# carlozamu/dynamic-video-compression-surveillance

Hardware: NVIDIA B200
Metric: 1080p_frames_per_second (higher is better)
Workload: dtype u8

## Files before the change

dynamic_video_compression_surveillance_b200/csrc/k_degrade4p.cuh:

```cuda
#pragma once
#include "k_degrade.cuh"

namespace dvc {

struct QuantP {
    float rcp[3];
    float nqs[3];
    float o[3];
};

template <typename T>
DEVI void dct4_fwd_t(T& x0, T& x1, T& x2, T& x3) {
    const T c1 = splat<T>(DVC_C1), c3 = splat<T>(DVC_C3), nc1 = splat<T>(-DVC_C1);
    const T s0 = add(x0, x3), s1 = add(x1, x2), d0 = sub(x0, x3), d1 = sub(x1, x2);
    x0 = add(s0, s1);
    x2 = sub(s0, s1);
    x1 = fma_(c3, d1, mul(c1, d0));
    x3 = fma_(c3, d0, mul(nc1, d1));
}
template <typename T>
DEVI void dct4_inv_t(T& x0, T& x1, T& x2, T& x3) {
    const T c1 = splat<T>(DVC_C1), c3 = splat<T>(DVC_C3), nc1 = splat<T>(-DVC_C1);
    const T e0 = add(x0, x2), e1 = sub(x0, x2);
    const T o0 = fma_(c3, x3, mul(c1, x1));
// ... 422 lines not shown
        }
    }
    if (counters) {
#pragma unroll
        for (int o = 16; o > 0; o >>= 1) {
            n_motion += __shfl_xor_sync(0xffffffffu, n_motion, o);
            n_static += __shfl_xor_sync(0xffffffffu, n_static, o);
        }
        if ((threadIdx.x & 31) == 0) {
            if (n_motion) atomicAdd(&counters->motion_pixels, (unsigned long long)n_motion);
            if (n_static) atomicAdd(&counters->static_blocks, (unsigned long long)n_static);
        }
    }
}

struct K4Geom {
    int gp;
    int parts;
    int nb;
    int sp;
    int span_bytes;
    int mask_bytes;
};

struct K4SGeom {
    K4Geom g;
    int stages;
    int tiles_per_frame;
    int n_tiles;
    int stage_bytes;
    int ybuf_bytes;
};

constexpr int K4S_GROUPS = 2;
constexpr int K4S_THREADS = K4S_GROUPS * 256 + 32;
constexpr int K4S_ISSUERS = 2;

DEVI void mbar_wait(uint32_t bar, uint32_t parity) {
    uint32_t done = 0;
    while (!done) {
        asm volatile("{\n .reg .pred p;\n mbarrier.try_wait.parity.shared::cta.b64 p, [%1], %2;\n selp.u32 %0, 1, 0, p;\n}"
                     : "=r"(done) : "r"(bar), "r"(parity) : "memory");
    }
}
DEVI void mbar_arrive(uint32_t bar) { asm volatile("mbarrier.arrive.shared::cta.b64 _, [%0];" ::"r"(bar) : "memory"); }
DEVI void group_sync(int id) { asm volatile("bar.sync %0, 256;" ::"r"(id) : "memory"); }

struct K4Walk {
    int f, l, df, dl, tpf;
    DEVI void init(int t0, int step, int tiles_per_frame) {
        tpf = tiles_per_frame; f = t0 / tpf; l = t0 - f * tpf; df = step / tpf; dl = step - df * tpf;
    }
    DEVI void next() { f += df; l += dl; if (l >= tpf) { l -= tpf; ++f; } }
};
struct K4Tile { size_t span_off, mask_off; int nbv, g0, ng; };
DEVI K4Tile k4_tile(const K4Walk& wk, const K4Geom& g, int H, int W, int wpr) {
    const int gpr = W >> 3, nbr = H >> 2;
    K4Tile r;
    int br0;
    if (g.parts == 1) { br0 = wk.l * g.nb; r.nbv = min(g.nb, nbr - br0); r.g0 = 0; r.ng = gpr; }
    else { br0 = wk.l / g.parts; r.nbv = 1; r.g0 = (wk.l - br0 * g.parts) * g.gp; r.ng = min(g.gp, gpr - r.g0); }
    r.span_off = ((size_t)wk.f * H + (size_t)(br0 * 4)) * W * 3 + (size_t)r.g0 * 24;
    r.mask_off = ((size_t)wk.f * H + (size_t)(br0 * 4)) * wpr;
    return r;
}

__global__ void __launch_bounds__(K4S_THREADS, 1)
k_degrade4s(const uint8_t* __restrict__ frames, const uint32_t* __restrict__ over127,
            const uint32_t* __restrict__ nonzero, uint8_t* __restrict__ compressed, uint8_t* __restrict__ overlay,
            int H, int W, int wpr, QuantP qp, Counters* __restrict__ counters, K4SGeom sg) {
    extern __shared__ __align__(128) uint8_t k4_smem[];
    const K4Geom& g = sg.g;
    const uint32_t s0 = (uint32_t)__cvta_generic_to_shared(k4_smem);
    const int S = sg.stages;
    const uint32_t ybufs = s0 + (uint32_t)S * (uint32_t)sg.stage_bytes;
    const uint32_t bars = ybufs + (uint32_t)K4S_GROUPS * (uint32_t)sg.ybuf_bytes;
    const uint32_t desc = (bars + 8u * (uint32_t)(2 * S) + 15u) & ~15u;
    const int tid = threadIdx.x;
    const int first = blockIdx.x, stride = gridDim.x;
    const int nj = first < sg.n_tiles ? (sg.n_tiles - first + stride - 1) / stride : 0;
    const uint32_t pitch = (uint32_t)W * 3u;
    const uint32_t mrow_bytes = (uint32_t)wpr * 4u;
    const bool contiguous = g.parts == 1;

    if (tid == 0) {
        for (int s = 0; s < S; ++s) {
            asm volatile("mbarrier.init.shared::cta.b64 [%0], 1;" ::"r"(bars + 8u * s));
            asm volatile("mbarrier.init.shared::cta.b64 [%0], %1;" ::"r"(bars + 8u * (S + s)), "r"(K4S_ISSUERS));
        }
        asm volatile("fence.mbarrier_init.release.cluster;" ::: "memory");
    }
    __syncthreads();

    if (tid >= K4S_GROUPS * 256) {
        if (tid > K4S_GROUPS * 256) return;
        K4Walk wl;
        wl.init(first, stride, sg.tiles_per_frame);
        for (int j = 0; j < nj; ++j) {
            const int s = j % S;
            const K4Tile t = k4_tile(wl, g, H, W, wpr);
            wl.next();
            const uint32_t sX = s0 + (uint32_t)s * (uint32_t)sg.stage_bytes;
            const uint32_t sMh = sX + g.span_bytes, sMn = sMh + g.mask_bytes;
            const uint32_t full = bars + 8u * s;
            const uint32_t mbytes = (uint32_t)(4 * t.nbv) * mrow_bytes;
            const uint32_t rows = contiguous ? (uint32_t)(4 * t.nbv) : 4u;
            const uint32_t rbytes = contiguous ? pitch : (uint32_t)t.ng * 24u;
            if (j >= S) mbar_wait(bars + 8u * (S + s), (uint32_t)(j / S - 1) & 1u);
            asm volatile("st.shared.v4.b32 [%0], {%1, %2, %3, %4};" ::"r"(desc + 16u * s), "r"(t.nbv), "r"(t.g0), "r"(t.ng), "r"(0) : "memory");
            asm volatile("mbarrier.arrive.expect_tx.shared::cta.b64 _, [%0], %1;" ::"r"(full), "r"(rows * rbytes + 2u * mbytes) : "memory");
            if (contiguous) bulk_load(sX, frames + t.span_off, rows * rbytes, full);
            else
                for (uint32_t r = 0; r < rows; ++r) bulk_load(sX + r * g.sp, frames + t.span_off + (size_t)r * pitch, rbytes, full);
            bulk_load(sMh, over127 + t.mask_off, mbytes, full);
            bulk_load(sMn, nonzero + t.mask_off, mbytes, full);
        }
        return;
    }

    const int grp = tid >> 8, t = tid & 255;
    const bool issuer = t < K4S_ISSUERS;
    const int gpr = W >> 3;
    int brl = 0, gxl = t;
    if (contiguous) { brl = t / gpr; gxl = t - brl * gpr; }
    const uint32_t toff = (uint32_t)(brl * 4) * (uint32_t)g.sp + (uint32_t)gxl * 24u;
    const uint32_t sY = ybufs + (uint32_t)grp * (uint32_t)sg.ybuf_bytes;
    unsigned n_motion = 0, n_static = 0;
    K4Walk ws;
    ws.init(first + grp * stride, K4S_GROUPS * stride, sg.tiles_per_frame);
    int s_prev = -1;
    for (int j = grp; j < nj; j += K4S_GROUPS) {
        const int s = j % S;
        const uint32_t sX = s0 + (uint32_t)s * (uint32_t)sg.stage_bytes;
        const uint32_t sMh = sX + g.span_bytes, sMn = sMh + g.mask_bytes;
        mbar_wait(bars + 8u * s, (uint32_t)(j / S) & 1u);
        uint32_t nbv, tg0, tng, unused;
        asm volatile("ld.shared.v4.b32 {%0, %1, %2, %3}, [%4];" : "=r"(nbv), "=r"(tg0), "=r"(tng), "=r"(unused) : "r"(desc + 16u * s));
        const bool active = brl < (int)nbv && gxl < (int)tng;
        uint32_t w[4][6];
        if (active) {
            const uint32_t moff = (uint32_t)(brl * 4) * mrow_bytes + tg0 + (uint32_t)gxl;
#pragma unroll
            for (int r = 0; r < 4; ++r)
#pragma unroll
                for (int i = 0; i < 3; ++i) lds64(sX + toff + r * g.sp + 8 * i, w[r][2 * i], w[r][2 * i + 1]);
            uint32_t hi[4], nz = 0;
#pragma unroll
            for (int r = 0; r < 4; ++r) {
                hi[r] = lds_u8(sMh + moff + r * mrow_bytes);
                nz |= lds_u8(sMn + moff + r * mrow_bytes);
            }
            if (overlay) {
#pragma unroll
                for (int r = 0; r < 4; ++r) {
                    if (hi[r] == 0u) continue;
                    uint32_t o[6];
#pragma unroll
                    for (int i = 0; i < 6; ++i) o[i] = w[r][i];
#pragma unroll
                    for (int b = 0; b < 2; ++b) {
                        const uint32_t m = hi[r] >> (4 * b);
                        if (m & 1u) { o[3 * b] = (o[3 * b] & 0xff000000u) | 0x00ff0000u; }
                        if (m & 2u) { o[3 * b] &= 0x00ffffffu; o[3 * b + 1] = (o[3 * b + 1] & 0xffff0000u) | 0x0000ff00u; }
                        if (m & 4u) { o[3 * b + 1] &= 0x0000ffffu; o[3 * b + 2] = (o[3 * b + 2] & 0xffffff00u) | 0x000000ffu; }
                        if (m & 8u) { o[3 * b + 2] = (o[3 * b + 2] & 0x000000ffu) | 0xff000000u; }
                    }
#pragma unroll
                    for (int i = 0; i < 3; ++i) sts64(sX + toff + r * g.sp + 8 * i, o[2 * i], o[2 * i + 1]);
                }
            }
            n_motion += __popc(hi[0]) + __popc(hi[1]) + __popc(hi[2]) + __popc(hi[3]);
            const bool st_a = (nz & 0xfu) == 0u, st_b = (nz >> 4) == 0u;
            n_static += (st_a ? 1u : 0u) + (st_b ? 1u : 0u);
            if (compressed) k4_blocks(w, st_a, st_b, qp);
        }
        if (issuer && s_prev >= 0) {
            asm volatile("cp.async.bulk.wait_group.read 0;" ::: "memory");
            mbar_arrive(bars + 8u * (S + s_prev));
        }
        group_sync(1 + grp);
        if (compressed && active) {
#pragma unroll
            for (int r = 0; r < 4; ++r)
#pragma unroll
                for (int i = 0; i < 3; ++i) sts64(sY + toff + r * g.sp + 8 * i, w[r][2 * i], w[r][2 * i + 1]);
        }
        asm volatile("fence.proxy.async.shared::cta;" ::: "memory");
        group_sync(1 + grp);
        if (issuer) {
            uint8_t* dst = t == 0 ? overlay : compressed;
            if (dst) {
                const K4Tile tl = k4_tile(ws, g, H, W, wpr);
                const uint32_t src = t == 0 ? sX : sY;
                if (contiguous) bulk_store(dst + tl.span_off, src, 4u * nbv * pitch);
                else
                    for (uint32_t r = 0; r < 4; ++r) bulk_store(dst + tl.span_off + (size_t)r * pitch, src + r * g.sp, tng * 24u);
            }
            asm volatile("cp.async.bulk.commit_group;" ::: "memory");
            s_prev = s;
        }
        ws.next();
    }
    if (issuer) asm volatile("cp.async.bulk.wait_group.read 0;" ::: "memory");
    if (counters) {
#pragma unroll
        for (int o = 16; o > 0; o >>= 1) {
            n_motion += __shfl_xor_sync(0xffffffffu, n_motion, o);
            n_static += __shfl_xor_sync(0xffffffffu, n_static, o);
        }
        if ((tid & 31) == 0) {
            if (n_motion) atomicAdd(&counters->motion_pixels, (unsigned long long)n_motion);
            if (n_static) atomicAdd(&counters->static_blocks, (unsigned long long)n_static);
        }
    }
}

}
// ... 1 lines not shown
```

dynamic_video_compression_surveillance_b200/csrc/k_mask.cuh:

```cuda
#pragma once
#include "common.cuh"
#include "k_front.cuh"

namespace dvc {

constexpr int WINDOW_MAX = 127;
struct MinCounts { uint8_t v[128]; };

template <int CB>
DEVI void bs_add(uint32_t (&c)[CB], uint32_t x) {
#pragma unroll
    for (int i = 0; i < CB; ++i) { uint32_t t = c[i] & x; c[i] ^= x; x = t; }
}
template <int CB>
DEVI void bs_sub(uint32_t (&c)[CB], uint32_t x) {
#pragma unroll
    for (int i = 0; i < CB; ++i) { uint32_t t = ~c[i] & x; c[i] ^= x; x = t; }
}
template <int CB>
DEVI uint32_t bs_ge(const uint32_t (&c)[CB], uint32_t m) {
    if (m >= (1u << CB)) return 0u;
    uint32_t ge = 0xffffffffu;
#pragma unroll
    for (int i = 0; i < CB; ++i) ge = ((m >> i) & 1u) ? (c[i] & ge) : (c[i] | ge);
    return ge;
}

template <int CNT_BITS>
__global__ void __launch_bounds__(256)
k_window_vote(const uint32_t* __restrict__ ring, int ring_cap, int H, int W, int wpr, long long f0, int slot0, int T,
              int K, const __grid_constant__ MinCounts mc, uint32_t* __restrict__ voted, int seg_len) {
    __shared__ uint8_t s_mc[128];
    if (threadIdx.x < 128) s_mc[threadIdx.x] = mc.v[threadIdx.x];
    __syncthreads();
    const size_t plane_words = (size_t)H * wpr;
    const size_t idx = (size_t)blockIdx.x * blockDim.x + threadIdx.x;
    if (idx >= plane_words) return;
    ring += (size_t)blockIdx.z * ring_cap * plane_words;
    voted += (size_t)blockIdx.z * T * plane_words;
    const int t0 = blockIdx.y * seg_len, t1 = min(T, t0 + seg_len);
    const uint32_t vm = valid_mask((int)(idx % wpr), W);
    uint32_t c[CNT_BITS] = {};
    const long long fs = f0 + t0;
    int s_new = (slot0 + t0) % ring_cap;
    const int nh = (int)min((long long)(K - 1), fs);
    int s = s_new - nh;
    if (s < 0) s += ring_cap;
    for (int i = 0; i < nh; ++i) {
        bs_add(c, ring[(size_t)s * plane_words + idx]);
        s = s + 1 == ring_cap ? 0 : s + 1;
    }
    int s_old = s_new - K;
    if (s_old < 0) s_old += ring_cap;
    int L = nh;
    constexpr int PF = 8;
    for (int tb = t0; tb < t1; tb += PF) {
        uint32_t w_new[PF], w_old[PF];
        int sn = s_new, so = s_old;
#pragma unroll
        for (int u = 0; u < PF; ++u) {
            const bool live = tb + u < t1;
            w_new[u] = live ? ring[(size_t)sn * plane_words + idx] : 0u;
            const bool evict = live && (L + u >= K) && (tb + u > t0);
            w_old[u] = evict ? ring[(size_t)so * plane_words + idx] : 0u;
            sn = sn + 1 == ring_cap ? 0 : sn + 1;
            so = so + 1 == ring_cap ? 0 : so + 1;
        }
#pragma unroll
        for (int u = 0; u < PF; ++u) {
            const int t = tb + u;
            if (t < t1) {
                if (L == K) { if (t > t0) bs_sub(c, w_old[u]); }
                else ++L;
                bs_add(c, w_new[u]);
                voted[(size_t)t * plane_words + idx] = bs_ge(c, s_mc[L - 1]) & vm;
            }
        }
        s_new = sn; s_old = so;
    }
}

template <int K>
__global__ void __launch_bounds__(256)
k_gray_diff_vote(const uint8_t* __restrict__ frames, int T, int H, int W, const uint8_t* __restrict__ prev_gray_in,
                 uint8_t* __restrict__ gray_state_out, uint32_t* __restrict__ ring, int wpr, int ring_cap, long long f0,
                 uint32_t thr, int seg_len, const __grid_constant__ MinCounts mc, uint32_t* __restrict__ voted) {
    const int gpr = W >> 4;
    const long long gid = (long long)blockIdx.x * blockDim.x + threadIdx.x;
    if (gid >= (long long)gpr * H) return;
    const int y = (int)(gid / gpr), gx = (int)(gid % gpr), x0 = gx << 4;
    const int t0 = blockIdx.y * seg_len, t1 = min(T, t0 + seg_len);
    const size_t frame_bytes = (size_t)H * W * 3, plane_bytes = (size_t)H * W, plane_words = (size_t)H * wpr;
    const size_t row_off = (size_t)y * W * 3 + (size_t)x0 * 3, px_off = (size_t)y * W + x0;
    {
        const size_t s = blockIdx.z;
        frames += s * T * frame_bytes;
        prev_gray_in += s * plane_bytes;
        if (gray_state_out) gray_state_out += s * plane_bytes;
        ring += s * ring_cap * plane_words;
        voted += s * T * plane_words;
    }
    uint16_t* const ring16 = reinterpret_cast<uint16_t*>(ring) + (size_t)y * wpr * 2 + gx;
    uint16_t* const vote16 = reinterpret_cast<uint16_t*>(voted) + (size_t)y * wpr * 2 + gx;
    auto gray_of_frame = [&](int t, uint32_t (&g)[4]) {
        const uint8_t* fr = frames + (size_t)t * frame_bytes + row_off;
        uint32_t w[12];
        load16(fr, *reinterpret_cast<uint32_t(*)[4]>(&w[0]));
        load16(fr + 16, *reinterpret_cast<uint32_t(*)[4]>(&w[4]));
        load16(fr + 32, *reinterpret_cast<uint32_t(*)[4]>(&w[8]));
        gray16_dp2a(w, g);
    };
    uint32_t hst[4] = {0u, 0u, 0u, 0u};
    uint32_t c[4] = {0u, 0u, 0u, 0u};
    auto push = [&](uint32_t b) {
        hst[3] = __funnelshift_l(hst[2], hst[3], 16); hst[2] = __funnelshift_l(hst[1], hst[2], 16);
        hst[1] = __funnelshift_l(hst[0], hst[1], 16); hst[0] = (hst[0] << 16) | b;
    };
    auto add = [&](uint32_t x) {
#pragma unroll
        for (int i = 0; i < 4; ++i) { const uint32_t tt = c[i] & x; c[i] ^= x; x = tt; }
    };
    auto sub = [&](uint32_t x) {
#pragma unroll
        for (int i = 0; i < 4; ++i) { const uint32_t tt = ~c[i] & x; c[i] ^= x; x = tt; }
    };
    const long long fs = f0 + t0;
    int nin = (int)min((long long)(K - 1), fs);
    uint32_t pg[4];
    if (t0 == 0) {
        load16(prev_gray_in + px_off, pg);
        for (int i = nin; i >= 1; --i) {
            const uint32_t b = ring16[(size_t)((f0 - i) % ring_cap) * plane_words * 2];
            push(b); add(b);
        }
    } else {
        gray_of_frame(t0 - nin - 1, pg);
        for (int t = t0 - nin; t < t0; ++t) {
            uint32_t g[4];
            gray_of_frame(t, g);
            const uint32_t b = diff_gt_bits16(g, pg, thr);
#pragma unroll
            for (int q = 0; q < 4; ++q) pg[q] = g[q];
            push(b); add(b);
        }
    }
    for (int t = t0; t < t1; ++t) {
        uint32_t g[4];
        gray_of_frame(t, g);
        const uint32_t b = diff_gt_bits16(g, pg, thr);
#pragma unroll
        for (int q = 0; q < 4; ++q) pg[q] = g[q];
        if (nin == K) sub((hst[(K - 1) >> 1] >> (((K - 1) & 1) * 16)) & 0xffffu);
        else ++nin;
        add(b);
        push(b);
        const uint32_t m = mc.v[nin - 1];
        uint32_t ge = 0u;
        if (m < 16u) {
            ge = 0xffffu;
#pragma unroll
            for (int i = 0; i < 4; ++i) ge = ((m >> i) & 1u) ? (c[i] & ge) : (c[i] | ge);
        }
        const size_t slot = (size_t)((f0 + t) % ring_cap);
        ring16[slot * plane_words * 2] = (uint16_t)b;
        vote16[(size_t)t * plane_words * 2] = (uint16_t)ge;
    }
    if (t1 == T && gray_state_out) store16(gray_state_out + px_off, pg);
}

template <bool ALIGNED, int PX = 16>
#ifndef DVC_EMA_MINB
#define DVC_EMA_MINB 4
#endif
__global__ void __launch_bounds__(256, PX == 8 ? DVC_EMA_MINB : 1)
k_ema(uint8_t* __restrict__ acc, const uint32_t* __restrict__ dilated, uint32_t* __restrict__ over127,
      uint32_t* __restrict__ nonzero, uint8_t* __restrict__ acc_all, int T, int H, int W, int wpr, float alpha,
      float beta) {
    static_assert(PX == 16 || PX == 8, "k_ema: 8 or 16 pixels per thread");
    constexpr int NQ = PX / 4;
    __shared__ uint8_t s_lut[512];
    {
        const float on = __fmul_rn(255.0f, beta);
        for (int i = threadIdx.x; i < 512; i += blockDim.x) {
            const float sv = __fmaf_rn((float)(i & 255), alpha, (i >> 8) ? on : 0.0f);
            s_lut[i] = (uint8_t)max(0, min(255, __float2int_rn(sv)));
        }
    }
    __syncthreads();
    const int gpr = (W + PX - 1) / PX;
    const long long gid = (long long)blockIdx.x * blockDim.x + threadIdx.x;
    if (gid >= (long long)gpr * H) return;
    const int y = (int)(gid / gpr), gx = (int)(gid % gpr), x0 = gx * PX;
    const size_t plane_words = (size_t)H * wpr, plane_bytes = (size_t)H * W;
    const int npx = min(PX, W - x0);
    {
        const size_t s = blockIdx.y;
        acc += s * plane_bytes;
        dilated += s * T * plane_words; over127 += s * T * plane_words; nonzero += s * T * plane_words;
        if (acc_all) acc_all += s * T * plane_bytes;
    }
    uint32_t a[NQ];
    uint8_t* arow = acc + (size_t)y * W;
    if (ALIGNED) {
        if (PX == 16) { uint4 t = *reinterpret_cast<const uint4*>(arow + x0); a[0] = t.x; a[1] = t.y; a[NQ - 2] = t.z; a[NQ - 1] = t.w; }
        else { uint2 t = *reinterpret_cast<const uint2*>(arow + x0); a[0] = t.x; a[1] = t.y; }
    } else { for (int i = 0; i < NQ; ++i) a[i] = 0; for (int i = 0; i < npx; ++i) a[i >> 2] |= (uint32_t)arow[x0 + i] << ((i & 3) * 8); }
    auto piece = [&](int t) -> uint32_t {
        const size_t wo = (size_t)t * plane_words + (size_t)y * wpr;
        return PX == 16 ? (uint32_t)reinterpret_cast<const uint16_t*>(dilated + wo)[gx] : (uint32_t)reinterpret_cast<const uint8_t*>(dilated + wo)[gx];
    };
    auto step = [&](int t, uint32_t bits) {
        const size_t woff = (size_t)t * plane_words + (size_t)y * wpr;
        uint32_t hi = 0, nz = 0, any = bits;
#pragma unroll
        for (int q = 0; q < NQ; ++q) any |= a[q];
        if (any != 0u) {
#pragma unroll
            for (int q = 0; q < NQ; ++q) {
                uint32_t nw = 0;
#pragma unroll
                for (int p = 0; p < 4; ++p) {
                    const int i = q * 4 + p;
                    const uint32_t v = s_lut[(((bits >> i) & 1u) << 8) | ((a[q] >> (8 * p)) & 0xffu)];
                    nw |= v << (8 * p);
                }
                a[q] = nw;
                hi |= ((((nw >> 7) & 0x01010101u) * 0x00204081u >> 21) & 0xfu) << (4 * q);
                nz |= (((((nw | ((nw & 0x7f7f7f7fu) + 0x7f7f7f7fu)) & 0x80808080u) >> 7) * 0x00204081u >> 21) & 0xfu) << (4 * q);
            }
            if (npx < PX) { const uint32_t m = (1u << npx) - 1u; hi &= m; nz &= m; }
        }
        if (PX == 16) {
            reinterpret_cast<uint16_t*>(over127 + woff)[gx] = (uint16_t)hi;
            reinterpret_cast<uint16_t*>(nonzero + woff)[gx] = (uint16_t)nz;
        } else {
            reinterpret_cast<uint8_t*>(over127 + woff)[gx] = (uint8_t)hi;
            reinterpret_cast<uint8_t*>(nonzero + woff)[gx] = (uint8_t)nz;
        }
        if (acc_all) {
            uint8_t* o = acc_all + (size_t)t * plane_bytes + (size_t)y * W;
            if (ALIGNED) {
                if (PX == 16) *reinterpret_cast<uint4*>(o + x0) = make_uint4(a[0], a[1], a[NQ - 2], a[NQ - 1]);
                else *reinterpret_cast<uint2*>(o + x0) = make_uint2(a[0], a[1]);
            } else for (int i = 0; i < npx; ++i) o[x0 + i] = (uint8_t)(a[i >> 2] >> ((i & 3) * 8));
        }
    };
    constexpr int PF = PX == 8 ? 8 : 1;
    int t = 0;
// ... 267 lines not shown
                case 115: rect_pass<15>(A, B, cx, flip); swap = false; break;
                case 117: rect_pass<17>(A, B, cx, flip); swap = false; break;
                case 119: rect_pass<19>(A, B, cx, flip); swap = false; break;
                case 121: rect_pass<21>(A, B, cx, flip); swap = false; break;
                case 123: rect_pass<23>(A, B, cx, flip); swap = false; break;
                case 125: rect_pass<25>(A, B, cx, flip); swap = false; break;
                case 127: rect_pass<27>(A, B, cx, flip); swap = false; break;
                case 129: rect_pass<29>(A, B, cx, flip); swap = false; break;
                case 131: rect_pass<31>(A, B, cx, flip); swap = false; break;
                case 133: rect_pass<33>(A, B, cx, flip); swap = false; break;
                case 1: small_pass<1, 3, 0>(A, B, cx, flip); break;
                case 2: small_pass<1, 7, 1>(A, B, cx, flip); break;
                case 3: ellipse2x2_pass(A, B, cx, flip); break;
                default: break;
            }
            if (swap) { uint32_t* t = A; A = B; B = t; }
            continue;
        }
        if (P.separable) {
            const HRun hr = make_hrun(P.lo[0], P.hi[0]);
            {
                const uint32_t* row = A + ra * wpr;
                uint32_t* out = B + ra * wpr + j;
                for (int r = ra; r < rb; ++r, row += wpr, out += wpr) {
                    const uint32_t p = (row[jp] ^ flip) & pm, c = (row[j] ^ flip) & vm, n = (row[jn] ^ flip) & nm;
                    *out = (p | c | n) ? hrun_or(p, c, n, hr) & vm : 0u;
                }
            }
            __syncthreads();
            const int dy0 = P.dy[0], dy1 = P.dy[P.nrows - 1];
            for (int r = ra; r < rb; ++r) {
                const int a0 = max(r + dy0, r_lo), a1 = min(r + dy1, r_hi - 1);
                const uint32_t* q = B + a0 * wpr + j;
                uint32_t acc = 0;
#pragma unroll 4
                for (int rr = a0; rr <= a1; ++rr, q += wpr) acc |= *q;
                A[r * wpr + j] = (acc ^ flip) & vm;
            }
            __syncthreads();
        } else if (P.small) {
            const int f_up = P.small_rows[0], f_mid = P.small_rows[1], f_dn = P.small_rows[2];
            const bool need_l = ((f_up | f_mid | f_dn) & 2) != 0, need_r = ((f_up | f_mid | f_dn) & 4) != 0;
            uint32_t pend = 0, up_prev = 0;
            const uint32_t* row = A + (ra - 1) * wpr;
            uint32_t* out = B + (ra - 1) * wpr + j;
            if (ra < rb)
                for (int x = ra - 1; x <= rb; ++x, row += wpr, out += wpr) {
                    uint32_t v_up = 0, v_mid = 0, v_dn = 0;
                    if (x >= r_lo && x < r_hi) {
                        const uint32_t c = (row[j] ^ flip) & vm;
                        const uint32_t cl = need_l ? __funnelshift_l((row[jp] ^ flip) & pm, c, 1) : 0u;
                        const uint32_t cr = need_r ? __funnelshift_r(c, (row[jn] ^ flip) & nm, 1) : 0u;
                        v_up = ((f_up & 1) ? c : 0u) | ((f_up & 2) ? cl : 0u) | ((f_up & 4) ? cr : 0u);
                        v_mid = ((f_mid & 1) ? c : 0u) | ((f_mid & 2) ? cl : 0u) | ((f_mid & 4) ? cr : 0u);
                        v_dn = ((f_dn & 1) ? c : 0u) | ((f_dn & 2) ? cl : 0u) | ((f_dn & 4) ? cr : 0u);
                    }
                    if (x > ra) out[-wpr] = ((pend | v_dn) ^ flip) & vm;
                    pend = up_prev | v_mid;
                    up_prev = v_up;
                }
            __syncthreads();
            uint32_t* t = A; A = B; B = t;
        } else {
            const int nrows = P.nrows;
            for (int r = ra; r < rb; ++r) {
                uint32_t acc = 0;
                for (int k = 0; k < nrows; ++k) {
                    const int rr = r + P.dy[k];
                    if (rr < r_lo || rr >= r_hi) continue;
                    const uint32_t* row = A + rr * wpr;
                    const uint32_t p = (row[jp] ^ flip) & pm, c = (row[j] ^ flip) & vm, n = (row[jn] ^ flip) & nm;
                    if (p | c | n) acc |= hrun_or(p, c, n, make_hrun(P.lo[k], P.hi[k]));
                }
                B[r * wpr + j] = (acc ^ flip) & vm;
            }
            __syncthreads();
            uint32_t* t = A; A = B; B = t;
        }
    }
    const int out_rows = min(band_rows, H - y0);
    for (int i = tid; i < out_rows * wpr; i += nt) dp[(size_t)y0 * wpr + i] = A[ch.halo_top * wpr + i];
}

}
```

dynamic_video_compression_surveillance_b200/csrc/dvc_b200.cu:

```cuda
#include <cuda_runtime.h>

#include <algorithm>
#include <cmath>
#include <cstdarg>
#include <cstdio>
#include <cstdlib>
#include <cstring>
#include <mutex>
#include <vector>

#include "../../include/dvc_b200.h"
#include "k_ccl.cuh"
#include "k_ccl_sweep.cuh"
#include "k_degrade.cuh"
#include "k_degrade4p.cuh"
#include "k_flow.cuh"
#include "k_front.cuh"
#include "k_mask.cuh"

using namespace dvc;

static thread_local char g_err[512] = "";

static int set_err(char* dst, int code, const char* fmt, ...) {
// ... 59 lines not shown
            p.small_rows[p.dy[i] + 1] = (int8_t)(1 | (p.lo[i] == -1 ? 2 : 0) | (p.hi[i] == 1 ? 4 : 0));
    p.kind = 0;
    if (sep && shape == DVC_SHAPE_RECT && (k & 1) && k >= 3) p.kind = (int16_t)(100 + k);
    if (small && p.small_rows[0] == 1 && p.small_rows[1] == 3 && p.small_rows[2] == 0) p.kind = 1;
    if (small && p.small_rows[0] == 1 && p.small_rows[1] == 7 && p.small_rows[2] == 1) p.kind = 2;
    return true;
}

static bool chain_push(MorphChain& ch, int op, int shape, int k) {
    auto push = [&](bool erode) {
        if (ch.n > 0 && shape == DVC_SHAPE_RECT && (k & 1) && k >= 3) {
            MorphPrim& q = ch.p[ch.n - 1];
            const int kq = q.kind - 100;
            if (q.kind >= 103 && (bool)q.erode == erode && kq + k - 1 <= MORPH_MAX_K) {
                if (!make_prim(DVC_SHAPE_RECT, kq + k - 1, erode, q)) return false;
                ch.halo_top += k / 2;
                ch.halo_bot += k / 2;
                ch.pad = std::max<int>(ch.pad, (kq + k - 1) / 2);
                return true;
            }
        }
        if (ch.n > 0 && shape == DVC_SHAPE_ELLIPSE && k == 2) {
            MorphPrim& q = ch.p[ch.n - 1];
            if (q.kind == 1 && (bool)q.erode == erode) {
                q.kind = 3;
                ch.halo_top += 1;
                return true;
            }
        }
        if (ch.n >= MORPH_MAX_PRIMS) return false;
        MorphPrim& p = ch.p[ch.n];
        if (!make_prim(shape, k, erode, p)) return false;
        ch.halo_top += -std::min<int>(p.dy[0], 0);
        ch.halo_bot += std::max<int>(p.dy[p.nrows - 1], 0);
        if (p.kind >= 100) ch.pad = std::max<int>(ch.pad, (p.kind - 100) / 2);
        ++ch.n;
        return true;
    };
    switch (op) {
        case DVC_MORPH_ERODE: return push(true);
        case DVC_MORPH_DILATE: return push(false);
        case DVC_MORPH_OPEN: return push(true) && push(false);
        case DVC_MORPH_CLOSE: return push(false) && push(true);
    }
    return false;
}

static void window_min_counts(double alpha, int K, MinCounts& mc) {
    memset(&mc, 0, sizeof(mc));
    for (int L = 1; L <= K; ++L) {
        const double rhs = alpha * L * 255;
        int c = 0;
        while (!((double)(c * 255) >= rhs) && c <= L) ++c;
        mc.v[L - 1] = (uint8_t)std::min(c, 255);
    }
}

#ifdef DVC_MEASURE
static int measure_env(const char* name, int dflt) { const char* e = getenv(name); return e ? atoi(e) : dflt; }
#else
static constexpr int measure_env(const char*, int dflt) { return dflt; }
#endif

struct PerDeviceOnce {
    std::mutex mu;
    bool done[64] = {};
    struct Guard {
        PerDeviceOnce* o; int d;
        explicit operator bool() const { return o != nullptr; }
        void commit() { o->done[d] = true; }
        ~Guard() { if (o) o->mu.unlock(); }
    };
    Guard begin() {
        int d = 0;
        cudaGetDevice(&d);
        d &= 63;
        mu.lock();
        if (done[d]) { mu.unlock(); return Guard{nullptr, d}; }
        return Guard{this, d};
    }
};

static int g_morph_smem_limit = 0;
static PerDeviceOnce g_morph_once;

static int launch_morph_chain(char* ERRBUF, const uint32_t* src, uint32_t* dst, int n, int H, int W,
                              const MorphChain& ch, cudaStream_t st) {
    const int wpr = words_per_row(W);
    if (ch.n == 0) {
        if (src != dst) CU(cudaMemcpyAsync(dst, src, (size_t)n * H * wpr * 4, cudaMemcpyDeviceToDevice, st));
        return DVC_OK;
    }
    if (auto once = g_morph_once.begin()) {
        int dev = 0, lim = 0;
        CU(cudaGetDevice(&dev));
        CU(cudaDeviceGetAttribute(&lim, cudaDevAttrMaxSharedMemoryPerBlockOptin, dev));
        CU(cudaFuncSetAttribute(k_morph_chain<256>, cudaFuncAttributeMaxDynamicSharedMemorySize, lim));
        CU(cudaFuncSetAttribute(k_morph_chain<1024>, cudaFuncAttributeMaxDynamicSharedMemorySize, lim));
        g_morph_smem_limit = lim;
        once.commit();
    }
    const int halo = ch.halo_top + ch.halo_bot;
    for (int i = 0; i < ch.n; ++i)
        for (int k = 0; k < ch.p[i].nrows; ++k)
            if (ch.p[i].lo[k] > 0 || ch.p[i].hi[k] < 0)
                return set_err(ERRBUF, DVC_ERR_UNSUPPORTED, "structuring element row that does not span its anchor column");
    if (wpr > 256) return set_err(ERRBUF, DVC_ERR_UNSUPPORTED, "frames wider than 8192 pixels are not supported by the morphology kernel");
    const size_t row_bytes = 2 * (size_t)wpr * 4;
    const size_t limit = (size_t)g_morph_smem_limit - 64;
    static const int target_kb = std::max(4, measure_env("DVC_MORPH_SMEM_KB", 36));
    const int pad = 2 * ch.pad;
    int band = (int)((size_t)target_kb * 1024 / row_bytes) - halo;
    if (band < 2 * halo) band = (int)(limit / row_bytes) - halo - pad;
    band = std::max(band, 16);
    band = std::min<int>(band, (int)(limit / row_bytes) - halo - pad);
    if (band < 1) return set_err(ERRBUF, DVC_ERR_UNSUPPORTED, "morphology chain halo %d rows x %d words does not fit in shared memory", halo, wpr);
    band = std::min(band, H);
    const int nbands = (H + band - 1) / band;
    band = (H + nbands - 1) / nbands;
    const size_t smem = 2 * (size_t)(band + halo + pad) * wpr * 4 + 16;
    const int threads = smem > 110 * 1024 ? 1024 : smem > 72 * 1024 ? 512 : 256;
    dim3 grid(nbands, n);
    if (threads == 256) k_morph_chain<256><<<grid, 256, smem, st>>>(src, dst, H, W, wpr, band, ch);
    else k_morph_chain<1024><<<grid, threads, smem, st>>>(src, dst, H, W, wpr, band, ch);
    CHECK_LAUNCH();
    return DVC_OK;
}

struct CclScratch {
    int *pa0 = nullptr, *paov = nullptr, *pb0 = nullptr, *pbov = nullptr, *ar0 = nullptr, *arov = nullptr;
    uint8_t* rowflag = nullptr;
    uint32_t* filled = nullptr;
    int *gp = nullptr, *ga = nullptr;
    size_t g_stride = 0;
    bool sweep = false;
    int frames = 0;
};

static PerDeviceOnce g_sweep_once;
static int g_sweep_smem_limit = 0;

static bool ccl_sweep_usable(int H, int W) {
    static const bool on = measure_env("DVC_CCL_SWEEP", 1) != 0;
    return on && W <= 8192 && ccl_sweep_smem_bytes(H, W) <= 200 * 1024;
}

static int launch_contour_sweep(char* ERRBUF, const uint32_t* raw, uint32_t* out, int n, int H, int W, int thr,
                                const CclScratch& sc, cudaStream_t st) {
    if (auto once = g_sweep_once.begin()) {
        int dev = 0, lim = 0;
        CU(cudaGetDevice(&dev));
        CU(cudaDeviceGetAttribute(&lim, cudaDevAttrMaxSharedMemoryPerBlockOptin, dev));
        CU(cudaFuncSetAttribute(k_ccl_sweep<1>, cudaFuncAttributeMaxDynamicSharedMemorySize, lim - 1024));
        CU(cudaFuncSetAttribute(k_ccl_sweep<2>, cudaFuncAttributeMaxDynamicSharedMemorySize, lim - 1024));
        CU(cudaFuncSetAttribute(k_ccl_sweep<4>, cudaFuncAttributeMaxDynamicSharedMemorySize, lim - 1024));
        g_sweep_smem_limit = lim;
        once.commit();
    }
    const int wpr = words_per_row(W);
    const size_t pw = (size_t)H * wpr, smem = ccl_sweep_smem_bytes(H, W);
    static const int chunk_rows = std::max(1, measure_env("DVC_CCL_ROWS", 16));
    if (smem + 2048 > (size_t)g_sweep_smem_limit) return set_err(ERRBUF, DVC_ERR_UNSUPPORTED, "contour filter: %d rows do not fit in shared memory", H);
    for (int i0 = 0; i0 < n; i0 += sc.frames) {
        const int m = std::min(sc.frames, n - i0);
        const uint32_t* r = raw + (size_t)i0 * pw;
        uint32_t* o = out + (size_t)i0 * pw;
        if (W <= 2048) k_ccl_sweep<1><<<m, SW_THREADS, smem, st>>>(r, o, sc.gp, sc.ga, sc.g_stride, H, W, wpr, thr, chunk_rows);
        else if (W <= 4096) k_ccl_sweep<2><<<m, SW_THREADS, smem, st>>>(r, o, sc.gp, sc.ga, sc.g_stride, H, W, wpr, thr, chunk_rows);
        else k_ccl_sweep<4><<<m, SW_THREADS, smem, st>>>(r, o, sc.gp, sc.ga, sc.g_stride, H, W, wpr, thr, chunk_rows);
        CHECK_LAUNCH();
    }
    return DVC_OK;
}

static int launch_contour_filter(char* ERRBUF, const uint32_t* raw, uint32_t* out, int n, int H, int W,
                                 double min_area, const CclScratch& sc, cudaStream_t st) {
    const int wpr = words_per_row(W);
    const size_t pw = (size_t)H * wpr;
    const double t2 = std::floor(2.0 * min_area);
    const int thr = t2 >= 2147483647.0 ? 2147483647 : (t2 < -1.0 ? -1 : (int)t2);
    if (sc.sweep) return launch_contour_sweep(ERRBUF, raw, out, n, H, W, thr, sc, st);
    for (int i0 = 0; i0 < n; i0 += sc.frames) {
        const int m = std::min(sc.frames, n - i0);
// ... 1490 lines not shown
```

Measured before the change: 203,100.

## Skip duplicate mask bulk load and software-pipeline frame loads in vote kernel

The degrade kernel now detects when the over127 and nonzero mask pointers alias and issues only one bulk mask copy, pointing both shared-memory views at it. This halves mask traffic in that case. The temporal vote kernel is restructured into a three-buffer rotation that prefetches raw frame bytes two steps ahead, overlapping global loads with the gray/diff/count work. It also replaces the per-step ring-slot modulo with an incrementing counter. This costs more registers and adds branchier loop control.

Result: faster. 205,700 (median of 6 runs) (+1.3%).

```diff
diff --git a/dynamic_video_compression_surveillance_b200/csrc/k_degrade4p.cuh b/dynamic_video_compression_surveillance_b200/csrc/k_degrade4p.cuh
--- a/dynamic_video_compression_surveillance_b200/csrc/k_degrade4p.cuh
+++ b/dynamic_video_compression_surveillance_b200/csrc/k_degrade4p.cuh
@@ -528,6 +528,7 @@
     const uint32_t pitch = (uint32_t)W * 3u;
     const uint32_t mrow_bytes = (uint32_t)wpr * 4u;
     const bool contiguous = g.parts == 1;
+    const bool one_mask = over127 == nonzero;
 
     if (tid == 0) {
         for (int s = 0; s < S; ++s) {
@@ -554,12 +555,12 @@
             const uint32_t rbytes = contiguous ? pitch : (uint32_t)t.ng * 24u;
             if (j >= S) mbar_wait(bars + 8u * (S + s), (uint32_t)(j / S - 1) & 1u);
             asm volatile("st.shared.v4.b32 [%0], {%1, %2, %3, %4};" ::"r"(desc + 16u * s), "r"(t.nbv), "r"(t.g0), "r"(t.ng), "r"(0) : "memory");
-            asm volatile("mbarrier.arrive.expect_tx.shared::cta.b64 _, [%0], %1;" ::"r"(full), "r"(rows * rbytes + 2u * mbytes) : "memory");
+            asm volatile("mbarrier.arrive.expect_tx.shared::cta.b64 _, [%0], %1;" ::"r"(full), "r"(rows * rbytes + (one_mask ? 1u : 2u) * mbytes) : "memory");
             if (contiguous) bulk_load(sX, frames + t.span_off, rows * rbytes, full);
             else
                 for (uint32_t r = 0; r < rows; ++r) bulk_load(sX + r * g.sp, frames + t.span_off + (size_t)r * pitch, rbytes, full);
             bulk_load(sMh, over127 + t.mask_off, mbytes, full);
-            bulk_load(sMn, nonzero + t.mask_off, mbytes, full);
+            if (!one_mask) bulk_load(sMn, nonzero + t.mask_off, mbytes, full);
         }
         return;
     }
@@ -578,7 +579,7 @@
     for (int j = grp; j < nj; j += K4S_GROUPS) {
         const int s = j % S;
         const uint32_t sX = s0 + (uint32_t)s * (uint32_t)sg.stage_bytes;
-        const uint32_t sMh = sX + g.span_bytes, sMn = sMh + g.mask_bytes;
+        const uint32_t sMh = sX + g.span_bytes, sMn = one_mask ? sMh : sMh + g.mask_bytes;
         mbar_wait(bars + 8u * s, (uint32_t)(j / S) & 1u);
         uint32_t nbv, tg0, tng, unused;
         asm volatile("ld.shared.v4.b32 {%0, %1, %2, %3}, [%4];" : "=r"(nbv), "=r"(tg0), "=r"(tng), "=r"(unused) : "r"(desc + 16u * s));
diff --git a/dynamic_video_compression_surveillance_b200/csrc/k_mask.cuh b/dynamic_video_compression_surveillance_b200/csrc/k_mask.cuh
--- a/dynamic_video_compression_surveillance_b200/csrc/k_mask.cuh
+++ b/dynamic_video_compression_surveillance_b200/csrc/k_mask.cuh
@@ -102,13 +102,11 @@
     }
     uint16_t* const ring16 = reinterpret_cast<uint16_t*>(ring) + (size_t)y * wpr * 2 + gx;
     uint16_t* const vote16 = reinterpret_cast<uint16_t*>(voted) + (size_t)y * wpr * 2 + gx;
-    auto gray_of_frame = [&](int t, uint32_t (&g)[4]) {
+    auto load_frame = [&](int t, uint32_t (&w)[12]) {
         const uint8_t* fr = frames + (size_t)t * frame_bytes + row_off;
-        uint32_t w[12];
         load16(fr, *reinterpret_cast<uint32_t(*)[4]>(&w[0]));
         load16(fr + 16, *reinterpret_cast<uint32_t(*)[4]>(&w[4]));
         load16(fr + 32, *reinterpret_cast<uint32_t(*)[4]>(&w[8]));
-        gray16_dp2a(w, g);
     };
     uint32_t hst[4] = {0u, 0u, 0u, 0u};
     uint32_t c[4] = {0u, 0u, 0u, 0u};
@@ -126,7 +124,8 @@
     };
     const long long fs = f0 + t0;
     int nin = (int)min((long long)(K - 1), fs);
-    uint32_t pg[4];
+    uint32_t pg[4] = {0u, 0u, 0u, 0u};
+    int ta = t0;
     if (t0 == 0) {
         load16(prev_gray_in + px_off, pg);
         for (int i = nin; i >= 1; --i) {
@@ -134,22 +133,19 @@
             push(b); add(b);
         }
     } else {
-        gray_of_frame(t0 - nin - 1, pg);
-        for (int t = t0 - nin; t < t0; ++t) {
-            uint32_t g[4];
-            gray_of_frame(t, g);
-            const uint32_t b = diff_gt_bits16(g, pg, thr);
-#pragma unroll
-            for (int q = 0; q < 4; ++q) pg[q] = g[q];
-            push(b); add(b);
-        }
-    }
-    for (int t = t0; t < t1; ++t) {
+        ta = t0 - nin - 1;
+    }
+    int slot = (int)(fs % ring_cap);
+    auto step = [&](int t, const uint32_t (&w)[12]) {
         uint32_t g[4];
-        gray_of_frame(t, g);
+        gray16_dp2a(w, g);
         const uint32_t b = diff_gt_bits16(g, pg, thr);
 #pragma unroll
         for (int q = 0; q < 4; ++q) pg[q] = g[q];
+        if (t < t0) {
+            if (t > ta) { push(b); add(b); }
+            return;
+        }
         if (nin == K) sub((hst[(K - 1) >> 1] >> (((K - 1) & 1) * 16)) & 0xffffu);
         else ++nin;
         add(b);
@@ -161,9 +157,22 @@
 #pragma unroll
             for (int i = 0; i < 4; ++i) ge = ((m >> i) & 1u) ? (c[i] & ge) : (c[i] | ge);
         }
-        const size_t slot = (size_t)((f0 + t) % ring_cap);
-        ring16[slot * plane_words * 2] = (uint16_t)b;
+        ring16[(size_t)slot * plane_words * 2] = (uint16_t)b;
         vote16[(size_t)t * plane_words * 2] = (uint16_t)ge;
+        slot = slot + 1 == ring_cap ? 0 : slot + 1;
+    };
+    uint32_t wa[12], wb[12], wc[12];
+    load_frame(ta, wa);
+    if (ta + 1 < t1) load_frame(ta + 1, wb);
+    for (int t = ta; t < t1; t += 3) {
+        if (t + 2 < t1) load_frame(t + 2, wc);
+        step(t, wa);
+        if (t + 1 == t1) break;
+        if (t + 3 < t1) load_frame(t + 3, wa);
+        step(t + 1, wb);
+        if (t + 2 == t1) break;
+        if (t + 4 < t1) load_frame(t + 4, wb);
+        step(t + 2, wc);
     }
     if (t1 == T && gray_state_out) store16(gray_state_out + px_off, pg);
 }
```

## Add warp-streaming morphology kernel for close-open plus odd dilation chains

Applied to the files above, without the earlier changes.

Adds a specialized kernel for recognized morphology chains: an optional fixed close/open prefix followed by a single KxK dilation (odd K up to 15) or the identity. Each warp streams down a band of rows and keeps vertical window state in registers through a log-structured sliding OR, using warp shuffles for horizontal neighbours. This replaces the shared-memory banded kernel with its per-primitive __syncthreads passes. Band count is chosen so there are enough warps to fill the SMs. The cost is halo recomputation at band edges, redundant edge lanes per 30-word tile, and one template instantiation per K.

New measurement: 209,700 before, 219,700 after (median of 6 runs). 4.8% higher.

```diff
diff --git a/dynamic_video_compression_surveillance_b200/csrc/dvc_b200.cu b/dynamic_video_compression_surveillance_b200/csrc/dvc_b200.cu
--- a/dynamic_video_compression_surveillance_b200/csrc/dvc_b200.cu
+++ b/dynamic_video_compression_surveillance_b200/csrc/dvc_b200.cu
@@ -165,7 +165,32 @@
 };
 
 static int g_morph_smem_limit = 0;
+static int g_morph_sms = 0;
 static PerDeviceOnce g_morph_once;
+
+static bool morph_stream_signature(const MorphChain& ch, bool& co, int& k) {
+    const MorphPrim* p = ch.p;
+    co = ch.n >= 3 && p[0].kind == 1 && !p[0].erode && p[1].kind == 3 && p[1].erode && p[2].kind == 1 && !p[2].erode;
+    int i = co ? 3 : 0;
+    k = 1;
+    if (i < ch.n) {
+        const MorphPrim& q = p[i++];
+        if (q.erode) return false;
+        if (q.kind >= 103 && q.kind <= 115) k = q.kind - 100;
+        else if (!(q.kind == 0 && q.separable && q.nrows == 1 && q.lo[0] == 0 && q.hi[0] == 0)) return false;
+    }
+    return i == ch.n;
+}
+
+template <bool CO>
+static void launch_morph_stream(int k, dim3 grid, cudaStream_t st, const uint32_t* src, uint32_t* dst, int H, int W, int wpr,
+                                int band, int nbands, int tiles, long long nwarps) {
+    switch (k) {
+#define DVC_MS_CASE(KK) case KK: k_morph_stream<CO, KK><<<grid, 256, 0, st>>>(src, dst, H, W, wpr, band, nbands, tiles, nwarps); break;
+        DVC_MS_CASE(1) DVC_MS_CASE(3) DVC_MS_CASE(5) DVC_MS_CASE(7) DVC_MS_CASE(9) DVC_MS_CASE(11) DVC_MS_CASE(13) DVC_MS_CASE(15)
+#undef DVC_MS_CASE
+    }
+}
 
 static int launch_morph_chain(char* ERRBUF, const uint32_t* src, uint32_t* dst, int n, int H, int W,
                               const MorphChain& ch, cudaStream_t st) {
@@ -178,10 +203,29 @@
         int dev = 0, lim = 0;
         CU(cudaGetDevice(&dev));
         CU(cudaDeviceGetAttribute(&lim, cudaDevAttrMaxSharedMemoryPerBlockOptin, dev));
+        CU(cudaDeviceGetAttribute(&g_morph_sms, cudaDevAttrMultiProcessorCount, dev));
         CU(cudaFuncSetAttribute(k_morph_chain<256>, cudaFuncAttributeMaxDynamicSharedMemorySize, lim));
         CU(cudaFuncSetAttribute(k_morph_chain<1024>, cudaFuncAttributeMaxDynamicSharedMemorySize, lim));
         g_morph_smem_limit = lim;
         once.commit();
+    }
+    bool co;
+    int k;
+    if (morph_stream_signature(ch, co, k)) {
+        const int halo = (co ? 4 : 0) + 2 * (k / 2);
+        const int tiles = (wpr + 29) / 30;
+        const long long per_band = (long long)n * tiles, want = 32LL * g_morph_sms;
+        int nb = (H + std::max(16, 10 * halo) - 1) / std::max(16, 10 * halo);
+        if (per_band * nb < want)
+            nb = std::max(nb, (int)std::min<long long>((want + per_band - 1) / per_band, (H + std::max(8, 2 * halo) - 1) / std::max(8, 2 * halo)));
+        const int band = (H + nb - 1) / nb;
+        nb = (H + band - 1) / band;
+        const long long nwarps = per_band * nb;
+        const dim3 grid((unsigned)((nwarps + 7) / 8));
+        if (co) launch_morph_stream<true>(k, grid, st, src, dst, H, W, wpr, band, nb, tiles, nwarps);
+        else launch_morph_stream<false>(k, grid, st, src, dst, H, W, wpr, band, nb, tiles, nwarps);
+        CHECK_LAUNCH();
+        return DVC_OK;
     }
     const int halo = ch.halo_top + ch.halo_bot;
     for (int i = 0; i < ch.n; ++i)
diff --git a/dynamic_video_compression_surveillance_b200/csrc/k_mask.cuh b/dynamic_video_compression_surveillance_b200/csrc/k_mask.cuh
--- a/dynamic_video_compression_surveillance_b200/csrc/k_mask.cuh
+++ b/dynamic_video_compression_surveillance_b200/csrc/k_mask.cuh
@@ -597,4 +597,122 @@
     for (int i = tid; i < out_rows * wpr; i += nt) dp[(size_t)y0 * wpr + i] = A[ch.halo_top * wpr + i];
 }
 
-}
+template <int K>
+struct VWinOr {
+    static constexpr int C = K >= 32 ? 32 : K >= 16 ? 16 : K >= 8 ? 8 : K >= 4 ? 4 : K >= 2 ? 2 : 1;
+    static constexpr int L = C == 32 ? 5 : C == 16 ? 4 : C == 8 ? 3 : C == 4 ? 2 : C == 2 ? 1 : 0;
+    uint32_t lv[L > 0 ? L : 1][C > 1 ? C / 2 : 1];
+    uint32_t tl[K > C ? K - C : 1];
+    DEVI void clear() {
+#pragma unroll
+        for (int i = 0; i < L; ++i)
+#pragma unroll
+            for (int d = 0; d < (1 << i); ++d) lv[i][d] = 0u;
+#pragma unroll
+        for (int d = 0; d < K - C; ++d) tl[d] = 0u;
+    }
+    DEVI uint32_t push(uint32_t o) {
+#pragma unroll
+        for (int i = 0; i < L; ++i) {
+            const int s = 1 << i;
+            const uint32_t back = lv[i][s - 1];
+#pragma unroll
+            for (int d = s - 1; d > 0; --d) lv[i][d] = lv[i][d - 1];
+            lv[i][0] = o;
+            o |= back;
+        }
+        if (K > C) {
+            const uint32_t back = tl[K - C - 1];
+#pragma unroll
+            for (int d = K - C - 1; d > 0; --d) tl[d] = tl[d - 1];
+            tl[0] = o;
+            o |= back;
+        }
+        return o;
+    }
+};
+
+template <bool CO, int K>
+__global__ void __launch_bounds__(256, 4)
+k_morph_stream(const uint32_t* __restrict__ src, uint32_t* __restrict__ dst, int H, int W, int wpr, int band_rows, int nbands,
+               int tiles, long long nwarps) {
+    constexpr int R = K / 2;
+    constexpr int HT = (CO ? 4 : 0) + R;
+    static_assert((K & 1) && HT < 32 && R < 32, "k_morph_stream: odd K, reach below 32 bits on each side");
+    const long long gw = ((long long)blockIdx.x * blockDim.x + threadIdx.x) >> 5;
+    if (gw >= nwarps) return;
+    const int lane = threadIdx.x & 31;
+    const int tile = (int)(gw % tiles);
+    const long long rest = gw / tiles;
+    const int band = (int)(rest % nbands);
+    const size_t img = (size_t)(rest / nbands);
+    const int j = tile * 30 + lane - 1;
+    const uint32_t vm = (j >= 0 && j < wpr) ? valid_mask(j, W) : 0u;
+    const bool owner = lane >= 1 && lane <= 30 && j < wpr;
+    const int y0 = band * band_rows, y1 = min(H, y0 + band_rows);
+    const int ys = max(0, y0 - HT), ye = y1 + R;
+    const int jc = min(max(j, 0), wpr - 1);
+    const uint32_t* q = src + (img * H + ys) * wpr + jc;
+    uint32_t* o = dst + (img * H + y0) * wpr + jc;
+
+    uint32_t d1 = 0u, t2 = 0u, m2a = 0u, m2b = 0u, d3 = 0u;
+    VWinOr<K> vw;
+    vw.clear();
+    auto step = [&](uint32_t x, bool below) -> uint32_t {
+        uint32_t v = x & vm;
+        if (CO) {
+            uint32_t p = __shfl_up_sync(0xffffffffu, v, 1);
+            uint32_t res = (v | d1 | __funnelshift_l(p, v, 1)) & vm;
+            d1 = v;
+            const uint32_t m = ~res & vm;
+            p = __shfl_up_sync(0xffffffffu, m, 1);
+            const uint32_t t = m | __funnelshift_l(p, m, 1);
+            res = t | __funnelshift_l(p, m, 2) | t2 | m2b;
+            m2b = m2a; m2a = m; t2 = t;
+            v = ~res & vm;
+            p = __shfl_up_sync(0xffffffffu, v, 1);
+            res = (v | d3 | __funnelshift_l(p, v, 1)) & vm;
+            d3 = v;
+            v = res;
+        }
+        if (K > 1) {
+            const uint32_t p = __shfl_up_sync(0xffffffffu, v, 1), n = __shfl_down_sync(0xffffffffu, v, 1);
+            const uint32_t h = below ? 0u : hwin_or<K>(p, v, n) & vm;
+            v = vw.push(h);
+        }
+        return v;
+    };
+    constexpr int U = 4;
+    auto load = [&](uint32_t (&x)[U], int y) {
+#pragma unroll
+        for (int u = 0; u < U; ++u) {
+            x[u] = *q;
+            if (y + u + 1 < H) q += wpr;
+        }
+    };
+    auto walk = [&](const uint32_t (&x)[U], int y, bool check) {
+#pragma unroll
+        for (int u = 0; u < U; ++u) {
+            const int yy = y + u;
+            if (!check || yy < ye) {
+                const uint32_t v = step(x[u], check && yy >= H);
+                if (!check || yy - R >= y0) {
+                    if (owner) *o = v;
+                    o += wpr;
+                }
+            }
+        }
+    };
+    const int fast_end = min(ye, H);
+    uint32_t x[U], nx[U];
+    load(x, ys);
+    for (int y = ys; y < ye; y += U) {
+        if (y + U < ye) load(nx, y + U);
+        if (y - R >= y0 && y + U <= fast_end) walk(x, y, false);
+        else walk(x, y, true);
+#pragma unroll
+        for (int u = 0; u < U; ++u) x[u] = nx[u];
+    }
+}
+
+}
```
